# Symb0x76/ChineseChessZero

Measured on AMD Instinct MI355X. Metric: self-play MCTS simulations/sec, higher is better.
Workload: dtype u8 rules / f32 Q (reference CPU path) / f64 PUCT (net: fp16)

## Files before the change

chinesechesszero_amd/csrc/cczero.hip:

```cpp
#include "../../include/cczero.h"

#include <hip/hip_runtime.h>

#include <cmath>
#include <cstdarg>
#include <cstdio>
#include <cstdlib>
#include <cstddef>
#include <cstring>
#include <new>
#include <vector>

#include "cczero_kernels.h"
#include "cczero_history.h"
#include "cczero_mate.h"
#include "cczero_netops.h"
#include "cczero_conv.h"
#include "cczero_conv_small.h"
#include "cczero_conv_narrow.h"
#include "cczero_conv_g16.h"
#include "cczero_conv_g16e.h"
#include "cczero_heads.h"
#include "cczero_snapshot.h"

// ... 2302 lines not shown
    return 0;
}

int ccz_pack_conv_weights_g16_f16(void *stream, const void *w_dev, void *wp_dev, int32_t cin)
{
    if (!w_dev || !wp_dev || w_dev == wp_dev || (cin != 64 && cin != 128 && cin != 256)) return fail(-1, "ccz_pack_conv_weights_g16_f16: bad arguments (cin must be 64, 128 or 256, not in place)");
    if ((((uintptr_t)w_dev) | ((uintptr_t)wp_dev)) & 15) return fail(-1, "ccz_pack_conv_weights_g16_f16: pointers must be 16-byte aligned");
    const int n = 256 * 9 * (cin >> 3);
    hipLaunchKernelGGL(k_pack_conv_weights_g16, dim3((unsigned)((n + 255) / 256)), dim3(256), 0, (hipStream_t)stream, (const cv_half8 *)w_dev, (cv_half8 *)wp_dev, (int)cin);
    HIP_TRY(hipGetLastError());
    return 0;
}

int ccz_pack_live_planes_g16_f16(void *stream, const void *leaf_dev, void *x64_dev, int32_t n_boards, const int32_t *rows_dev, const int32_t *n_rows_dev)
{
    if (!leaf_dev || !x64_dev || n_boards < 0 || (!rows_dev) != (!n_rows_dev)) return fail(-1, "ccz_pack_live_planes_g16_f16: bad arguments");
    if ((uintptr_t)x64_dev & 15) return fail(-1, "ccz_pack_live_planes_g16_f16: output must be 16-byte aligned");
    if (n_boards == 0) return 0;
    hipLaunchKernelGGL(k_pack_live_planes, dim3((unsigned)n_boards), dim3(kPackThreads), 0, (hipStream_t)stream, (const _Float16 *)leaf_dev, (half8_t *)x64_dev, (int)n_boards,
                       (const int *)rows_dev, (const int *)n_rows_dev, rows_dev ? 3 : 1);
    HIP_TRY(hipGetLastError());
    return 0;
}

static int pack_planes128(const char *who, void *stream, const void *leaf_dev, void *x128_dev, int32_t n_boards, const int32_t *rows_dev, const int32_t *n_rows_dev, int flags)
{
    if (!leaf_dev || !x128_dev || n_boards < 0 || (!rows_dev) != (!n_rows_dev)) return fail(-1, "%s: bad arguments", who);
    if ((uintptr_t)x128_dev & 15) return fail(-1, "%s: output must be 16-byte aligned", who);
    if (n_boards == 0) return 0;
    hipLaunchKernelGGL(k_pack_planes128, dim3((unsigned)n_boards), dim3(kPackThreads), 0, (hipStream_t)stream, (const _Float16 *)leaf_dev, (half8_t *)x128_dev, (int)n_boards,
                       (const int *)rows_dev, (const int *)n_rows_dev, flags);
    HIP_TRY(hipGetLastError());
    return 0;
}

int ccz_pack_planes128_f16(void *stream, const void *leaf_dev, void *x128_dev, int32_t n_boards)
{
    return pack_planes128("ccz_pack_planes128_f16", stream, leaf_dev, x128_dev, n_boards, nullptr, nullptr, 0);
}

int ccz_pack_planes128_g16_f16(void *stream, const void *leaf_dev, void *x128_dev, int32_t n_boards, const int32_t *rows_dev, const int32_t *n_rows_dev)
{
    return pack_planes128("ccz_pack_planes128_g16_f16", stream, leaf_dev, x128_dev, n_boards, rows_dev, n_rows_dev, 1);
}

int ccz_pack_planes128_rows_f16(void *stream, const void *leaf_dev, void *x128_dev, int32_t n_boards, const int32_t *rows_dev, const int32_t *n_rows_dev)
{
    if (!rows_dev || !n_rows_dev) return fail(-1, "ccz_pack_planes128_rows_f16: bad arguments");
    return pack_planes128("ccz_pack_planes128_rows_f16", stream, leaf_dev, x128_dev, n_boards, rows_dev, n_rows_dev, 0);
}

int ccz_conv3x3_stem128_f16(void *stream, const void *x128_dev, const void *w_dev, const void *bias_f32_dev, void *y_dev, int64_t n_pixels, int32_t relu)
{
    if (relu & ~(3 | CCZ_CONV_G16)) return fail(-1, "ccz_conv3x3_stem128_f16: flags are ReLU (1), tile order (2) and CCZ_CONV_G16");
    return conv3x3_launch("ccz_conv3x3_stem128_f16", stream, x128_dev, w_dev, bias_f32_dev, nullptr, y_dev, n_pixels, relu, 128);
}

int ccz_conv3x3_stem128_f16_live(void *stream, const void *x128_dev, const void *w_dev, const void *bias_f32_dev, void *y_dev, int64_t n_pixels, int32_t relu,
                                 const int32_t *live_rows_dev, int32_t part, int32_t n_parts)
{
    if (relu & ~(3 | CCZ_CONV_G16)) return fail(-1, "ccz_conv3x3_stem128_f16_live: flags are ReLU (1), tile order (2) and CCZ_CONV_G16");
    if (!live_rows_dev || g16_bad_part(part, n_parts)) return fail(-1, "ccz_conv3x3_stem128_f16_live: null live-row count or bad part / n_parts");
    return conv3x3_launch("ccz_conv3x3_stem128_f16_live", stream, x128_dev, w_dev, bias_f32_dev, nullptr, y_dev, n_pixels, relu, 128, live_rows_dev, part | (n_parts << 16));
}

int ccz_pack_live_planes_f16(void *stream, const void *leaf_dev, void *x64_dev, int32_t n_boards)
{
    if (!leaf_dev || !x64_dev || n_boards < 0) return fail(-1, "ccz_pack_live_planes_f16: bad arguments");
    if ((uintptr_t)x64_dev & 15) return fail(-1, "ccz_pack_live_planes_f16: output must be 16-byte aligned");
    if (n_boards == 0) return 0;
    hipLaunchKernelGGL(k_pack_live_planes, dim3((unsigned)n_boards), dim3(kPackThreads), 0, (hipStream_t)stream, (const _Float16 *)leaf_dev, (half8_t *)x64_dev, (int)n_boards,
                       (const int *)nullptr, (const int *)nullptr, 0);
    HIP_TRY(hipGetLastError());
    return 0;
}

#ifdef CCZ_STAMPS
int ccz_debug_conv_stamps(unsigned long long *out_host)
{
    HIP_TRY(hipDeviceSynchronize());
    HIP_TRY(hipMemcpyFromSymbol(out_host, HIP_SYMBOL(g_cv_stamps), sizeof(unsigned long long) * 2048 * 2 * 16));
    return 0;
}
int ccz_debug_stamps(ccz_engine *e, void *stream, unsigned long long *out_host)
{
    NEED(e);
    hipStream_t s = (hipStream_t)stream;
    HIP_TRY(hipMemcpyAsync(out_host, e->d.stamps, (size_t)e->d.B * 16 * 8, hipMemcpyDeviceToHost, s));
    HIP_TRY(hipStreamSynchronize(s));
    return 0;
}
#endif

int ccz_heads_conv1x1_f16(void *stream, const void *x_dev, const void *w32_dev, const void *bias32_f32_dev, void *pol_dev, void *val_dev,
                          int32_t n_boards, int32_t flags, const int32_t *live_boards_dev)
{
    if (!x_dev || !w32_dev || !bias32_f32_dev || !pol_dev || !val_dev || n_boards < 0) return fail(-1, "ccz_heads_conv1x1_f16: bad arguments");
    if ((((uintptr_t)x_dev) | ((uintptr_t)w32_dev) | ((uintptr_t)bias32_f32_dev)) & 15) return fail(-1, "ccz_heads_conv1x1_f16: x, weights and bias must be 16-byte aligned");
    if (flags & ~CCZ_CONV_G16) return fail(-1, "ccz_heads_conv1x1_f16: unknown flags 0x%x", flags);
    const bool g16 = (flags & CCZ_CONV_G16) != 0;
    if (g16 && (n_boards & 15)) return fail(-1, "ccz_heads_conv1x1_f16: the group-of-16 layout holds whole groups of 16 boards (n_boards = %d)", n_boards);
    if (n_boards == 0) return 0;
    const long cells = ((long)n_boards * 90 + 15) / 16;
    const unsigned blocks = (unsigned)((cells + 3) / 4 < 768 ? (cells + 3) / 4 : 768);
    if (g16)
        hipLaunchKernelGGL(k_head_conv1x1<true>, dim3(blocks), dim3(256), 0, (hipStream_t)stream, (const _Float16 *)x_dev, (const _Float16 *)w32_dev,
                           (const float *)bias32_f32_dev, (_Float16 *)pol_dev, (_Float16 *)val_dev, (int)n_boards, (const int *)live_boards_dev);
    else
        hipLaunchKernelGGL(k_head_conv1x1<false>, dim3(blocks), dim3(256), 0, (hipStream_t)stream, (const _Float16 *)x_dev, (const _Float16 *)w32_dev,
                           (const float *)bias32_f32_dev, (_Float16 *)pol_dev, (_Float16 *)val_dev, (int)n_boards, (const int *)live_boards_dev);
    HIP_TRY(hipGetLastError());
    return 0;
}

static int conv3x3_cn_launch(const char *who, void *stream, const void *x_dev, const void *w_dev, const void *bias_f32_dev, const void *residual_dev, void *y_dev,
                             int64_t n_pixels, int32_t relu, int32_t cin, int32_t cout, const int32_t *live_rows_dev, int32_t row0)
{
    if ((cin != 64 && cin != 128) || (cout != 64 && cout != 128))
        return fail(-1, "%s: unsupported shape %d -> %d channels (cin and cout must be 64 or 128; 256-wide towers: ccz_conv3x3_c256_f16)", who, cin, cout);
    if (!x_dev || !w_dev || !bias_f32_dev || !y_dev || n_pixels < 0 || n_pixels > (int64_t)INT32_MAX / 256)
        return fail(-1, "%s: bad arguments (null pointer, or n_pixels outside 0 .. 2^31 / 256)", who);
    if ((((uintptr_t)x_dev) | ((uintptr_t)w_dev) | ((uintptr_t)bias_f32_dev) | ((uintptr_t)residual_dev) | ((uintptr_t)y_dev)) & 15)
        return fail(-1, "%s: pointers must be 16-byte aligned", who);
    if (x_dev == y_dev) return fail(-1, "%s: the output may alias the residual but not the input", who);
    if (relu & ~(CCZ_CONV_RELU | CCZ_CONV_DESCENDING | CCZ_CONV_FORCE_SMALL | CCZ_CONV_FORCE_TILE))
        return fail(-1, "%s: flags are ReLU, tile order and the two force bits (board-major rows only)", who);
    const bool whole = n_pixels % 90 == 0;
    if (live_rows_dev && !whole) return fail(-1, "%s: the live form takes whole boards (n_pixels = boards * 90)", who);
    if ((relu & CCZ_CONV_FORCE_SMALL) && (relu & CCZ_CONV_FORCE_TILE)) return fail(-1, "%s: both force bits set", who);
    if ((relu & CCZ_CONV_FORCE_SMALL) && (live_rows_dev || !whole)) return fail(-1, "%s: the small form takes whole boards and no live count", who);
    if (n_pixels == 0) return 0;
    const bool res = residual_dev != nullptr;
    const bool small = whole && !live_rows_dev && !(relu & CCZ_CONV_FORCE_TILE) && ((relu & CCZ_CONV_FORCE_SMALL) || n_pixels <= kSmallMaxPixels);
#define CCZ_CN_SMALL(RES_, CIN_, COUT_)                                                                                                         \
    hipLaunchKernelGGL((k_conv3x3_small<RES_, CIN_, COUT_>), dim3((unsigned)((n_pixels + kSmPix - 1) / kSmPix), COUT_ / 16), dim3(256), 0, (hipStream_t)stream, \
                       (const _Float16 *)x_dev, (const _Float16 *)w_dev, (const float *)bias_f32_dev, (const _Float16 *)residual_dev, (_Float16 *)y_dev, \
                       (int)n_pixels, (int)(relu & 1))
#define CCZ_CN_TILE(RES_, CIN_, COUT_)                                                                                                          \
    hipLaunchKernelGGL((k_conv3x3_narrow<RES_, CIN_, COUT_>), dim3((unsigned)((n_pixels + kNwBM - 1) / kNwBM)), dim3(512), 0, (hipStream_t)stream, \
                       (const _Float16 *)x_dev, (const _Float16 *)w_dev, (const float *)bias_f32_dev, (const _Float16 *)residual_dev, (_Float16 *)y_dev, \
                       (int)n_pixels, (int)(relu & 3), (const int *)live_rows_dev, (int)row0)
#define CCZ_CN_FORM(RES_, CIN_, COUT_) do { if (small) CCZ_CN_SMALL(RES_, CIN_, COUT_); else CCZ_CN_TILE(RES_, CIN_, COUT_); } while (0)
#define CCZ_CN_RES(CIN_, COUT_) do { if (res) CCZ_CN_FORM(true, CIN_, COUT_); else CCZ_CN_FORM(false, CIN_, COUT_); } while (0)
    if (cin == 64 && cout == 64) CCZ_CN_RES(64, 64);
    else if (cin == 64) CCZ_CN_RES(64, 128);
    else if (cout == 64) CCZ_CN_RES(128, 64);
    else CCZ_CN_RES(128, 128);
#undef CCZ_CN_RES
#undef CCZ_CN_FORM
#undef CCZ_CN_TILE
#undef CCZ_CN_SMALL
    HIP_TRY(hipGetLastError());
    return 0;
}

int ccz_conv3x3_cn_f16(void *stream, const void *x_dev, const void *w_dev, const void *bias_f32_dev, const void *residual_dev, void *y_dev,
                       int64_t n_pixels, int32_t relu, int32_t cin, int32_t cout)
{
    return conv3x3_cn_launch("ccz_conv3x3_cn_f16", stream, x_dev, w_dev, bias_f32_dev, residual_dev, y_dev, n_pixels, relu, cin, cout, nullptr, 0);
}

int ccz_conv3x3_cn_f16_live(void *stream, const void *x_dev, const void *w_dev, const void *bias_f32_dev, const void *residual_dev, void *y_dev,
                            int64_t n_pixels, int32_t relu, int32_t cin, int32_t cout, const int32_t *live_rows_dev, int32_t part, int32_t n_parts)
{
    if (!live_rows_dev || g16_bad_part(part, n_parts)) return fail(-1, "ccz_conv3x3_cn_f16_live: null live-row count or bad part / n_parts");
    return conv3x3_cn_launch("ccz_conv3x3_cn_f16_live", stream, x_dev, w_dev, bias_f32_dev, residual_dev, y_dev, n_pixels, relu, cin, cout, live_rows_dev,
// ... 78 lines not shown
```

chinesechesszero_amd/csrc/cczero_conv_g16.h:

```cpp
#pragma once
#include "cczero_conv.h"

namespace ccz {

constexpr int kG5Rows = 288;
constexpr int kG5SlabRows = 576;
constexpr int kG5SlabBytes = kG5SlabRows * 64;
constexpr int kG5WBytes = 256 * 64;
constexpr int kG5Ring = 5, kG5Ahead = 3;
constexpr int kG5AOff = kG5Ring * kG5WBytes;
constexpr int kG5Dump = kG5AOff + 2 * kG5SlabBytes;
constexpr int kG5Lds = kG5Dump + 8 * 1024;
constexpr int kG5ERow = 528;
static_assert(kG5Rows * kG5ERow <= kG5Dump, "epilogue image must fit the operand buffers");
constexpr int kG5QRows = 576;
constexpr int kG5QSlabRows = 864;
constexpr int kG5QSlabBytes = kG5QSlabRows * 64;
constexpr int kG5QWBytes = 128 * 64;
constexpr int kG5QAOff = kG5Ring * kG5QWBytes;
constexpr int kG5QDump = kG5QAOff + 2 * kG5QSlabBytes;
constexpr int kG5QLds = kG5QDump + 8 * 1024;
constexpr int kG5QERow = 272;
static_assert(kG5QLds == 159744 && kG5QLds <= kG5Lds, "quad tile: ring + two slabs + dump must fit the workgroup's LDS");
static_assert(kG5QRows * kG5QERow == 156672 && kG5QRows * kG5QERow <= kG5QLds,
              "quad tile: the epilogue image covers the operand buffers AND most of the dump area (free once every DMA has landed)");

constexpr int kG16CChunk = 1440 * 64;
__device__ __forceinline__ unsigned g16c_off(long p)
{
    const long g = p / 1440;
    return (unsigned)(g * (1440 * 512) + (p - g * 1440) * 64);
}

struct G5Ctx {
    unsigned char *lds;
    const _Float16 *X, *W;
    unsigned xbytes, wbytes;
    unsigned xbytes_part;
    unsigned xoff[5];
    unsigned xstep, whalf;
    unsigned woff;
    int zo[2], zd[2];
    int wave_dst;
    int lane16;
    int wave_dst_part, wave_step_part;
    int a_off;
    int vb[2];
    int cin, cmask;
};

__host__ __device__ constexpr bool g5_slab_tap(int t) { return t >= 1 && t <= 5; }
constexpr int kG5Split = 7;
__host__ __device__ constexpr int g5_dma(int t) { return 2 + (g5_slab_tap(t) ? 1 : 0); }
__host__ __device__ constexpr int g5_vmcnt(int t) { return g5_dma(t) + g5_dma(t - 1); }
static_assert(g5_vmcnt(0) == 4 && g5_vmcnt(1) == 5 && g5_vmcnt(2) == 6 && g5_vmcnt(3) == 6 && g5_vmcnt(4) == 6 && g5_vmcnt(5) == 6 &&
              g5_vmcnt(6) == 5 && g5_vmcnt(7) == 4 && g5_vmcnt(8) == 4, "g5_vmcnt table");
static_assert(g5_dma(0) == 2 && g5_dma(1) == 3 && g5_dma(2) == 3 && g5_dma(3) == 3 && g5_dma(4) == 3 && g5_dma(5) == 3 && g5_dma(6) == 2 &&
              g5_dma(7) == 2 && g5_dma(8) == 2, "23 DMA loads per chunk and thread: 5 slab pieces + 9 x 2 weight pieces");
__host__ __device__ constexpr int g5q_nslab(int t) { return t == 0 ? 2 : t <= 5 ? 1 : 0; }
__host__ __device__ constexpr int g5q_dma(int t) { return 1 + g5q_nslab(t); }
__host__ __device__ constexpr int g5q_vmcnt(int t) { return g5q_dma(t) + g5q_dma((t + 8) % 9); }
static_assert(g5q_vmcnt(0) == 4 && g5q_vmcnt(1) == 5 && g5q_vmcnt(2) == 4 && g5q_vmcnt(3) == 4 && g5q_vmcnt(4) == 4 && g5q_vmcnt(5) == 4 &&
              g5q_vmcnt(6) == 3 && g5q_vmcnt(7) == 2 && g5q_vmcnt(8) == 2, "g5q_vmcnt table");
static_assert(g5q_dma(0) == 3 && g5q_dma(1) == 2 && g5q_dma(2) == 2 && g5q_dma(3) == 2 && g5q_dma(4) == 2 && g5q_dma(5) == 2 && g5q_dma(6) == 1 &&
              g5q_dma(7) == 1 && g5q_dma(8) == 1, "16 DMA loads per chunk and thread: 7 slab pieces + 9 weight pieces");

template <int T, int N> __host__ __device__ constexpr bool g5_on_board()
{
    return !((T % 3 == 0 && N == 0) || (T % 3 == 2 && N == 8));
}

template <bool LDS_DONE = false> __device__ __forceinline__ void g5_barrier()
{
    if constexpr (LDS_DONE) asm volatile("s_waitcnt lgkmcnt(0)" ::: "memory");
    __builtin_amdgcn_sched_barrier(0);
    __builtin_amdgcn_s_barrier();
    __builtin_amdgcn_sched_barrier(0);
}

__device__ __forceinline__ void g5_zero_ranks(const G5Ctx &c, int buf)
{
    int l16 = c.lane16, zero = 0;
    asm volatile("" : "+v"(l16), "+v"(zero));
    typedef int g5_int4 __attribute__((ext_vector_type(4)));
    const g5_int4 z = {zero, zero, zero, zero};
#pragma unroll
    for (int j = 0; j < 2; ++j) *(g5_int4 *)(c.lds + (l16 + (c.zo[j] + buf * c.zd[j]))) = z;
    asm volatile("s_waitcnt lgkmcnt(0)" ::: "memory");
}

#define G5_CELL(TAP, N)                                                                                                   \
    {                                                                                                                     \
        if constexpr (TAP % 3 == 2)                                                                                       \
            b[N] = *(const cv_half8 *)(lds + c.vb[BUFn] + G5_REFILL(N) * 1024);                                           \
        if constexpr (g5_on_board<TAP, N>()) {                                                                            \
            constexpr int NB = N + TAP % 3 - 1;                                                                           \
            _Pragma("unroll") for (int i = 0; i < 4; ++i)                                                                 \
                acc[i][N] = __builtin_amdgcn_mfma_f32_16x16x32_f16(acur[i], b[NB], acc[i][N], 0, 0, 0);                   \
        }                                                                                                                 \
        __builtin_amdgcn_sched_barrier(0);                                                                                \
    }
#define G5_CELLS(TAP, LO, HI)                                                                                             \
    if constexpr (LO <= 0 && 0 < HI) G5_CELL(TAP, 0) if constexpr (LO <= 1 && 1 < HI) G5_CELL(TAP, 1) if constexpr (LO <= 2 && 2 < HI) G5_CELL(TAP, 2) \
    if constexpr (LO <= 3 && 3 < HI) G5_CELL(TAP, 3) if constexpr (LO <= 4 && 4 < HI) G5_CELL(TAP, 4) if constexpr (LO <= 5 && 5 < HI) G5_CELL(TAP, 5) \
    if constexpr (LO <= 6 && 6 < HI) G5_CELL(TAP, 6) if constexpr (LO <= 7 && 7 < HI) G5_CELL(TAP, 7) if constexpr (LO <= 8 && 8 < HI) G5_CELL(TAP, 8)

template <int J, bool Q = false, bool CM = false>
__device__ __forceinline__ void g5_step(const G5Ctx &c, cv_f32x4 (&acc)[4][9], int chunk, int &ring_rd, int &ring_wr,
                                         cv_half8 (&a0)[4], cv_half8 (&a1)[4], cv_half8 (&b)[9])
{
    constexpr int T = J % 9, BUF = J / 9;
    constexpr int Tn = (T + 1) % 9, BUFn = (T == 8) ? 1 - BUF : BUF;
    constexpr int kWB = Q ? kG5QWBytes : kG5WBytes, kAOff = Q ? kG5QAOff : kG5AOff, kSlab = Q ? kG5QSlabBytes : kG5SlabBytes;
    cv_half8 (&acur)[4] = (J & 1) ? a1 : a0;
    cv_half8 (&anxt)[4] = (J & 1) ? a0 : a1;
    unsigned char *const lds = c.lds;

#define G5_REFILL(N) (9 + N + 9 * (Tn / 3 - 1))
    constexpr int T2 = (T + kG5Ahead) % 9;
    const int chunk2 = chunk + (T + kG5Ahead >= 9 ? 1 : 0);
    G5_CELLS(T, 0, 1)
    if constexpr (Q && g5q_nslab(T) > 0) {
        constexpr int pass = T == 0 ? 0 : T + 1;
        const unsigned so = (unsigned)((chunk + 1) * (CM ? kG16CChunk : 64));
        const unsigned live = chunk < c.cmask ? (pass < 6 ? c.xbytes : c.xbytes_part) : 0u;
        cv_blds16(c.X, live, c.xoff[0], so + pass * c.xstep,
                  lds + (pass < 6 ? kAOff + (1 - BUF) * kSlab + pass * 8192 + c.wave_dst : c.wave_dst_part + (1 - BUF) * c.wave_step_part));
        if constexpr (g5q_nslab(T) > 1) cv_blds16(c.X, live, c.xoff[0], so + (pass + 1) * c.xstep, lds + kAOff + (1 - BUF) * kSlab + ((pass + 1) * 8192 + c.wave_dst));
        __builtin_amdgcn_sched_barrier(0);
    }
    if constexpr (!Q && g5_dma(T) > 2) {
        constexpr int pass = T - 1;
        const unsigned live = pass < 4 ? c.xbytes : c.xbytes_part;
        cv_blds16(c.X, chunk < c.cmask ? live : 0u, c.xoff[pass], (unsigned)((chunk + 1) * (CM ? kG16CChunk : 64)),
                  lds + (pass < 4 ? kG5AOff + (1 - BUF) * kG5SlabBytes + pass * 8192 + c.wave_dst : c.wave_dst_part + (1 - BUF) * c.wave_step_part));
        __builtin_amdgcn_sched_barrier(0);
    }
    G5_CELLS(T, 1, 2)
    if constexpr (Q) {
        cv_blds16(c.W, chunk2 <= c.cmask ? c.wbytes : 0u, c.woff, (unsigned)((T2 + 9 * chunk2) * (2 * 8192)) + c.whalf, lds + ring_wr * kWB + c.wave_dst);
        __builtin_amdgcn_sched_barrier(0);
        G5_CELLS(T, 2, 3)
    } else {
        const unsigned wlive = chunk2 <= c.cmask ? c.wbytes : 0u;
        const unsigned so = (unsigned)((T2 + 9 * chunk2) * (2 * 8192));
        unsigned char *const d = lds + ring_wr * kG5WBytes + c.wave_dst;
        cv_blds16(c.W, wlive, c.woff, so, d);
        __builtin_amdgcn_sched_barrier(0);
        G5_CELLS(T, 2, 3)
        cv_blds16(c.W, wlive, c.woff, so + 8192u, d + 8192);
        __builtin_amdgcn_sched_barrier(0);
    }
    G5_CELLS(T, 3, kG5Split)

    ring_rd = ring_rd + 1 == kG5Ring ? 0 : ring_rd + 1;
    cv_wait_vm<Q ? g5q_vmcnt(T) : g5_vmcnt(T)>();
    if constexpr (!Q && T == 7) g5_zero_ranks(c, 1 - BUF);
    g5_barrier();

    {
        const unsigned char *wa = lds + (ring_rd * kWB + c.a_off);
#pragma unroll
        for (int i = 0; i < 4; ++i) anxt[i] = *(const cv_half8 *)(wa + i * 1024);
        __builtin_amdgcn_sched_barrier(0);
    }
    G5_CELLS(T, kG5Split, 9)
    ring_wr = ring_wr + 1 == kG5Ring ? 0 : ring_wr + 1;
#undef G5_REFILL
}

struct G5Heads {
    const _Float16 *w32;
    const float *b32;
    _Float16 *pol, *val;
    int nb;
};

__device__ __forceinline__ void g5_heads_phase(const unsigned char *lds, int w, int lane, const G5Heads &ha, const long (&board0)[2],
                                               const int (&pos0)[2], bool skip1)
{
    const int r = lane & 15, q4 = lane >> 4;
    cv_half8 a[2][8];
#pragma unroll
    for (int m = 0; m < 2; ++m)
#pragma unroll
        for (int s = 0; s < 8; ++s) a[m][s] = *(const cv_half8 *)(ha.w32 + (m * 16 + r) * 256 + s * 32 + q4 * 8);
    const float4 b0 = *(const float4 *)(ha.b32 + 4 * q4), b1 = *(const float4 *)(ha.b32 + 16 + 4 * q4);
    for (int cell = w; cell < 18; cell += 8) {
        const unsigned char *row = lds + (cell * 16 + r) * kG5ERow + q4 * 16;
        cv_f32x4 acc0, acc1;
        acc0[0] = b0.x; acc0[1] = b0.y; acc0[2] = b0.z; acc0[3] = b0.w;
        acc1[0] = b1.x; acc1[1] = b1.y; acc1[2] = b1.z; acc1[3] = b1.w;
#pragma unroll
        for (int s = 0; s < 8; ++s) {
            const cv_half8 b = *(const cv_half8 *)(row + s * 64);
            acc0 = __builtin_amdgcn_mfma_f32_16x16x32_f16(a[0][s], b, acc0, 0, 0, 0);
            acc1 = __builtin_amdgcn_mfma_f32_16x16x32_f16(a[1][s], b, acc1, 0, 0, 0);
        }
        const int wnr = cell >= 9 ? 1 : 0, n = cell - 9 * wnr;
        const long board = board0[wnr] + r;
        if (board < ha.nb && !(skip1 && wnr)) {
            const int pos = pos0[wnr] + n;
            _Float16 *po = ha.pol + board * 1536 + pos * 17;
            _Float16 *vo = ha.val + board * 640 + pos * 7;
#pragma unroll
            for (int e = 0; e < 4; ++e) po[4 * q4 + e] = (_Float16)fmaxf(acc0[e], 0.0f);
            if (q4 == 0) {
                po[16] = (_Float16)fmaxf(acc1[0], 0.0f);
                vo[0] = (_Float16)fmaxf(acc1[1], 0.0f);
                vo[1] = (_Float16)fmaxf(acc1[2], 0.0f);
                vo[2] = (_Float16)fmaxf(acc1[3], 0.0f);
            } else if (q4 == 1) {
#pragma unroll
                for (int e = 0; e < 4; ++e) vo[3 + e] = (_Float16)fmaxf(acc1[e], 0.0f);
            }
        }
    }
}

__device__ __forceinline__ int g5_live_groups(const int *live_rows, int row0, int cap, int &first)
{
    const int part = row0 & 0xffff, n_parts = row0 >> 16;
    const int G = (*live_rows + 15) >> 4;
    const int per = (G + n_parts - 1) / n_parts;
    first = part * per;
    int live = G - first;
    live = live < 0 ? 0 : (live > per ? per : live);
    return live > cap ? cap : live;
}

template <bool RES, bool HEADS>
__device__ __forceinline__ void g5_live_part(int first, int cin, const _Float16 *__restrict__ &X, const _Float16 *&R, _Float16 *&Y, long &first_board)
{
    const long off = (long)first * 1440 * kCvC;
    X += (long)first * 1440 * cin;
    if (!HEADS) Y += off;
    if (RES) R += off;
    first_board = (long)first * 16;
}

__device__ __forceinline__ int g5_xcd_tile(int blk, int tiles, int flags)
{
    const int b = blk, x = b & 7, per = tiles >> 3, rem = tiles & 7;
    const int tile = x * per + (x < rem ? x : rem) + (b >> 3);
    return __builtin_amdgcn_readfirstlane((flags & 2) ? tiles - 1 - tile : tile);
}

__device__ __forceinline__ void g5_ctx_common(G5Ctx &c, unsigned char *lds, const _Float16 *X, const _Float16 *W, int w, unsigned xbytes, int cin, int chunks)
{
    c.lds = lds;
// ... 144 lines not shown
    cv_wait_vm<4>();
    g5_zero_ranks(c, 0);
    g5_barrier<true>();

    int ring_rd = 0, ring_wr = kG5Ahead;
    cv_half8 a0[4], a1[4], b[9];
#pragma unroll
    for (int i = 0; i < 4; ++i) a0[i] = *(const cv_half8 *)(lds + c.a_off + i * 1024);
#pragma unroll
    for (int n = 0; n < 9; ++n) b[n] = *(const cv_half8 *)(lds + c.vb[0] + (9 + n - 9) * 1024);
#define G5_S(j) g5_step<j, false, CM && !ONE>(c, acc, chunk + (j) / 9, ring_rd, ring_wr, a0, a1, b)
    if constexpr (ONE) {
        const int chunk = 0;
        G5_S(0); G5_S(1); G5_S(2); G5_S(3); G5_S(4); G5_S(5); G5_S(6); G5_S(7); G5_S(8);
    } else {
        for (int chunk = 0; chunk <= c.cmask; chunk += 2) {
            G5_S(0); G5_S(1); G5_S(2); G5_S(3); G5_S(4); G5_S(5); G5_S(6); G5_S(7); G5_S(8);
            G5_S(9); G5_S(10); G5_S(11); G5_S(12); G5_S(13); G5_S(14); G5_S(15); G5_S(16); G5_S(17);
        }
    }
#undef G5_S
    cv_wait_vm<0>();

    g5_barrier();
    const int lane_e = (int)__builtin_amdgcn_mbcnt_hi(~0u, __builtin_amdgcn_mbcnt_lo(~0u, 0u));
    const int re = lane_e & 15, q4e = lane_e >> 4;
    const int prow = lane_e >> 5, piece = lane_e & 31;
    const long pbase = p0 + w * 36 + prow;
    cv_half8 rv[18];
    g5_image_store<kG5ERow>(lds, acc, wm, wn, re, q4e);
    if constexpr (CM) {
        const int erow = g16c_lane_row(lane_e), ep = lane_e & 3;
        const size_t yo = (size_t)g16c_off(p0 + erow) + (size_t)(w * kG16CChunk + ep * 16);
        if (RES) {
#pragma unroll
            for (int it = 0; it < 18; ++it) rv[it] = *(const cv_half8 *)((const unsigned char *)R + yo + it * 1024);
        }
        g5_barrier<true>();
        g5c_rows_out<kG5ERow, RES, HEADS>(lds, erow * kG5ERow + w * 64 + ep * 16, yo, Y, relu, rv);
    } else {
        if (RES) {
#pragma unroll
            for (int it = 0; it < 18; ++it) rv[it] = *(const cv_half8 *)(R + (pbase + it * 2) * kCvC + piece * 8);
        }
        g5_barrier<true>();
        g5_rows_out<kG5ERow, 2, RES, HEADS>(lds, w * 36 + prow, piece, pbase, piece * 8, Y, relu, rv);
    }
    if constexpr (HEADS) {
        g5_barrier<true>();
        const long grp = p0 / 1440;
        const int rank0 = (int)((p0 - grp * 1440) / 144);
        const long board0[2] = {first_board + grp * 16, first_board + grp * 16};
        const int pos0[2] = {rank0 * 9, rank0 * 9 + 9};
        g5_heads_phase(lds, w, lane_e, ha, board0, pos0, false);
    }
}

template <bool RES, bool CM = false>
__device__ __forceinline__ void g5q_tile(unsigned char *lds, int blk, int grid, const _Float16 *__restrict__ X, const _Float16 *__restrict__ W,
                                         const float *__restrict__ bias, const _Float16 *R, _Float16 *Y, int M, int relu, int cin,
                                         const int *live_rows, int row0)
{
    const int tid = threadIdx.x, lane = tid & 63;
    const int w = __builtin_amdgcn_readfirstlane(tid >> 6);
    const int r = lane & 15, q4 = lane >> 4;
    const int wm = w & 1, wn = w >> 1;
    int tiles = grid;
    if (live_rows) {
        int first;
        const int live = g5_live_groups(live_rows, row0, M / 1440, first);
        M = live * 1440;
        tiles = live * 4;
        if (blk >= tiles) return;
        long first_board;
        g5_live_part<RES, false>(first, cin, X, R, Y, first_board);
    }
    const int tile = g5_xcd_tile(blk, tiles, relu);
    const int h = tile & 1;
    const long p0 = (long)(tile >> 2) * 1440 + 144 + (long)((tile >> 1) & 1) * kG5QRows;
    relu &= 1;

    G5Ctx c;
    g5_ctx_common(c, lds, X, W, w, (unsigned)M * (unsigned)cin * 2u, cin, cin >> 5);
    c.wave_dst_part = w < 6 ? kG5QAOff + 6 * 8192 + w * 1024 : kG5QDump + w * 1024;
    c.wave_step_part = w < 6 ? kG5QSlabBytes : 0;
    c.xbytes_part = w < 6 ? c.xbytes : 0u;
    c.xstep = CM ? 128u * 64u : 128u * (unsigned)cin * 2u;
    c.whalf = (unsigned)h * 8192u;
    {
        const int sr = tid >> 2, pos = tid & 3;
        const int schunk = pos ^ ((0 - (sr >> 2)) & 3);
        if constexpr (CM) c.xoff[0] = g16c_off(p0 - 144 + sr) + (unsigned)(schunk * 16);
        else c.xoff[0] = (unsigned)((p0 - 144 + sr) * cin + schunk * 8) * 2u;
        c.woff = (unsigned)(tid * 16);
    }
#pragma unroll
    for (int it = 0; it < 7; ++it)
        cv_blds16(X, it < 6 ? c.xbytes : c.xbytes_part, c.xoff[0], it * c.xstep, lds + (it < 6 ? kG5QAOff + it * 8192 + c.wave_dst : c.wave_dst_part));
#pragma unroll
    for (int u = 0; u < kG5Ahead; ++u) cv_blds16(W, c.wbytes, c.woff, (unsigned)(u * 2 * 8192) + c.whalf, lds + u * kG5QWBytes + c.wave_dst);
    g5_ctx_frags(c, r, q4, wm, wn * 9, kG5QAOff, kG5QSlabBytes);

    cv_f32x4 acc[4][9];
#pragma unroll
    for (int i = 0; i < 4; ++i) g5_acc_row_from_bias(acc[i], bias + h * 128 + wm * 64 + i * 16 + 4 * q4);

    cv_wait_vm<2>();
    g5_barrier();

    int ring_rd = 0, ring_wr = kG5Ahead;
    cv_half8 a0[4], a1[4], b[9];
#pragma unroll
    for (int i = 0; i < 4; ++i) a0[i] = *(const cv_half8 *)(lds + c.a_off + i * 1024);
#pragma unroll
    for (int n = 0; n < 9; ++n) b[n] = *(const cv_half8 *)(lds + c.vb[0] + n * 1024);
    for (int chunk = 0; chunk <= c.cmask; chunk += 2) {
#define G5Q_S(j) g5_step<j, true, CM>(c, acc, chunk + (j) / 9, ring_rd, ring_wr, a0, a1, b)
        G5Q_S(0); G5Q_S(1); G5Q_S(2); G5Q_S(3); G5Q_S(4); G5Q_S(5); G5Q_S(6); G5Q_S(7); G5Q_S(8);
        G5Q_S(9); G5Q_S(10); G5Q_S(11); G5Q_S(12); G5Q_S(13); G5Q_S(14); G5Q_S(15); G5Q_S(16); G5Q_S(17);
#undef G5Q_S
    }
    cv_wait_vm<0>();

    g5_barrier();
    const int lane_e = (int)__builtin_amdgcn_mbcnt_hi(~0u, __builtin_amdgcn_mbcnt_lo(~0u, 0u));
    const int re = lane_e & 15, q4e = lane_e >> 4;
    const int prow = lane_e >> 4, piece = lane_e & 15;
    const long pbase = p0 + w * 72 + prow;
    const int gcol = h * 128 + piece * 8;
    cv_half8 rv[18];
    g5_image_store<kG5QERow>(lds, acc, wm, wn, re, q4e);
    if constexpr (CM) {
        const int erow = g16c_lane_row(lane_e), ep = lane_e & 3, ch = w & 3, irow = (w >> 2) * 288 + erow;
        const size_t yo = (size_t)g16c_off(p0 + irow) + (size_t)((h * 4 + ch) * kG16CChunk + ep * 16);
        if (RES) {
#pragma unroll
            for (int it = 0; it < 18; ++it) rv[it] = *(const cv_half8 *)((const unsigned char *)R + yo + it * 1024);
        }
        g5_barrier<true>();
        g5c_rows_out<kG5QERow, RES, false>(lds, irow * kG5QERow + ch * 64 + ep * 16, yo, Y, relu, rv);
    } else {
        if (RES) {
#pragma unroll
            for (int it = 0; it < 18; ++it) rv[it] = *(const cv_half8 *)(R + (pbase + it * 4) * kCvC + gcol);
        }
        g5_barrier<true>();
        g5_rows_out<kG5QERow, 4, RES, false>(lds, w * 72 + prow, piece, pbase, gcol, Y, relu, rv);
    }
}

template <bool RES>
__global__ __launch_bounds__(512) void k_conv3x3_g16(const _Float16 *__restrict__ X, const _Float16 *__restrict__ W,
                                                         const float *__restrict__ bias, const _Float16 *R,
                                                         _Float16 *Y, int M, int relu, int cin, const int *live_rows, int row0)
{
    __shared__ __attribute__((aligned(16))) unsigned char lds[kG5Lds];
    g5_tile<RES, false>(lds, blockIdx.x, gridDim.x, X, W, bias, R, Y, M, relu, cin, live_rows, row0, G5Heads{});
}

template <bool RES>
__global__ __launch_bounds__(512) void k_conv3x3_g16_quad(const _Float16 *__restrict__ X, const _Float16 *__restrict__ W,
                                                            const float *__restrict__ bias, const _Float16 *R,
                                                            _Float16 *Y, int M, int relu, int cin, const int *live_rows, int row0)
{
    __shared__ __attribute__((aligned(16))) unsigned char lds[kG5Lds];
    g5q_tile<RES>(lds, blockIdx.x, gridDim.x, X, W, bias, R, Y, M, relu, cin, live_rows, row0);
}

__global__ __launch_bounds__(512) void k_conv3x3_g16_stem(const _Float16 *__restrict__ X, const _Float16 *__restrict__ W,
                                                            const float *__restrict__ bias, _Float16 *Y, int M, int relu, int cin,
                                                            const int *live_rows, int row0)
{
    __shared__ __attribute__((aligned(16))) unsigned char lds[kG5Lds];
    g5_tile<false, false, true>(lds, blockIdx.x, gridDim.x, X, W, bias, nullptr, Y, M, relu, cin, live_rows, row0, G5Heads{});
}

__global__ __launch_bounds__(512) void k_conv3x3_g16_heads(const _Float16 *__restrict__ X, const _Float16 *__restrict__ W,
                                                             const float *__restrict__ bias, const _Float16 *R, _Float16 *Y, int M,
                                                             int relu, int cin, const int *live_rows, int row0, G5Heads ha)
{
    __shared__ __attribute__((aligned(16))) unsigned char lds[kG5Lds];
    if (live_rows) ha.nb = *live_rows;
    g5_tile<true, true>(lds, blockIdx.x, gridDim.x, X, W, bias, R, Y, M, relu, cin, live_rows, row0, ha);
}

__global__ __launch_bounds__(512) void k_conv3x3_g16c_stem(const _Float16 *__restrict__ X, const _Float16 *__restrict__ W,
                                                             const float *__restrict__ bias, _Float16 *Y, int M, int relu, int cin,
                                                             const int *live_rows, int row0)
{
    __shared__ __attribute__((aligned(16))) unsigned char lds[kG5Lds];
    g5_tile<false, false, true, true>(lds, blockIdx.x, gridDim.x, X, W, bias, nullptr, Y, M, relu, cin, live_rows, row0, G5Heads{});
}

__global__ __launch_bounds__(512) void k_conv3x3_g16c_heads(const _Float16 *__restrict__ X, const _Float16 *__restrict__ W,
                                                              const float *__restrict__ bias, const _Float16 *R, _Float16 *Y, int M,
                                                              int relu, int cin, const int *live_rows, int row0, G5Heads ha)
{
    __shared__ __attribute__((aligned(16))) unsigned char lds[kG5Lds];
    if (live_rows) ha.nb = *live_rows;
    g5_tile<true, true, false, true>(lds, blockIdx.x, gridDim.x, X, W, bias, R, Y, M, relu, cin, live_rows, row0, ha);
}

__global__ __launch_bounds__(256) void k_pack_conv_weights_g16(const cv_half8 *__restrict__ w, cv_half8 *__restrict__ wp, int cin)
{
// ... 10 lines not shown
```

Baseline: 201,300.

## Halve quad-tile conv barriers by pairing half-steps with a six-slot weight ring

The quad-tile 3x3 conv main loop now waits and issues a workgroup barrier only on every second tap step. It grows the weight ring from five to six slots and prefetches four steps ahead, so that ring slots are compile-time functions of the step. Slab DMA issue is rescheduled across the 18 half-steps so each wait count still covers the data needed. This cuts barrier and vmcnt stall overhead in exchange for 2KB more LDS and deeper prefetch, with the dump area shifted for some waves. Stamp instrumentation and profiling scripts are added behind a compile flag.

```diff
diff --git a/chinesechesszero_amd/csrc/cczero.hip b/chinesechesszero_amd/csrc/cczero.hip
--- a/chinesechesszero_amd/csrc/cczero.hip
+++ b/chinesechesszero_amd/csrc/cczero.hip
@@ -2408,6 +2408,17 @@
     HIP_TRY(hipMemcpyFromSymbol(out_host, HIP_SYMBOL(g_cv_stamps), sizeof(unsigned long long) * 2048 * 2 * 16));
     return 0;
 }
+int ccz_debug_g5q_stamps(unsigned long long *out_host, int clear)
+{
+    HIP_TRY(hipDeviceSynchronize());
+    HIP_TRY(hipMemcpyFromSymbol(out_host, HIP_SYMBOL(g_g5q_stamps), sizeof(unsigned long long) * 4096 * 8 * 8));
+    if (clear) {
+        void *p = nullptr;
+        HIP_TRY(hipGetSymbolAddress(&p, HIP_SYMBOL(g_g5q_stamps)));
+        HIP_TRY(hipMemset(p, 0, sizeof(unsigned long long) * 4096 * 8 * 8));
+    }
+    return 0;
+}
 int ccz_debug_stamps(ccz_engine *e, void *stream, unsigned long long *out_host)
 {
     NEED(e);
diff --git a/chinesechesszero_amd/csrc/cczero_conv_g16.h b/chinesechesszero_amd/csrc/cczero_conv_g16.h
--- a/chinesechesszero_amd/csrc/cczero_conv_g16.h
+++ b/chinesechesszero_amd/csrc/cczero_conv_g16.h
@@ -17,13 +17,19 @@
 constexpr int kG5QSlabRows = 864;
 constexpr int kG5QSlabBytes = kG5QSlabRows * 64;
 constexpr int kG5QWBytes = 128 * 64;
-constexpr int kG5QAOff = kG5Ring * kG5QWBytes;
+#ifndef CCZ_G5Q_PAIR
+#define CCZ_G5Q_PAIR 1
+#endif
+constexpr bool kG5QPair = CCZ_G5Q_PAIR != 0;
+constexpr int kG5QRing = kG5QPair ? 6 : kG5Ring, kG5QAhead = kG5QPair ? 4 : kG5Ahead;
+constexpr int kG5QAOff = kG5QRing * kG5QWBytes;
 constexpr int kG5QDump = kG5QAOff + 2 * kG5QSlabBytes;
-constexpr int kG5QLds = kG5QDump + 8 * 1024;
+constexpr int kG5QDumpWave0 = kG5QPair ? 6 : 0;
+constexpr int kG5QLds = kG5QDump + (8 - kG5QDumpWave0) * 1024;
 constexpr int kG5QERow = 272;
-static_assert(kG5QLds == 159744 && kG5QLds <= kG5Lds, "quad tile: ring + two slabs + dump must fit the workgroup's LDS");
+static_assert(kG5QLds == (kG5QPair ? 161792 : 159744) && kG5QLds <= kG5Lds, "quad tile: ring + two slabs + dump must fit the workgroup's LDS");
 static_assert(kG5QRows * kG5QERow == 156672 && kG5QRows * kG5QERow <= kG5QLds,
-              "quad tile: the epilogue image covers the operand buffers AND most of the dump area (free once every DMA has landed)");
+              "quad tile: the epilogue image covers the operand buffers (ring of five: and most of the dump area), free once every DMA has landed");
 
 constexpr int kG16CChunk = 1440 * 64;
 __device__ __forceinline__ unsigned g16c_off(long p)
@@ -47,6 +53,9 @@
     int a_off;
     int vb[2];
     int cin, cmask;
+#ifdef CCZ_STAMPS
+    mutable unsigned long long st_vm, st_bar, st_n;
+#endif
 };
 
 __host__ __device__ constexpr bool g5_slab_tap(int t) { return t >= 1 && t <= 5; }
@@ -65,6 +74,17 @@
 static_assert(g5q_dma(0) == 3 && g5q_dma(1) == 2 && g5q_dma(2) == 2 && g5q_dma(3) == 2 && g5q_dma(4) == 2 && g5q_dma(5) == 2 && g5q_dma(6) == 1 &&
               g5q_dma(7) == 1 && g5q_dma(8) == 1, "16 DMA loads per chunk and thread: 7 slab pieces + 9 weight pieces");
 
+__host__ __device__ constexpr int g5q2_nslab(int j) { return j < 9 ? g5q_nslab(j) : j - 9 <= 1 ? 2 : j - 9 <= 4 ? 1 : 0; }
+__host__ __device__ constexpr int g5q2_pass(int j) { return j % 9 == 0 ? 0 : g5q2_pass(j - 1) + g5q2_nslab(j - 1); }
+__host__ __device__ constexpr int g5q2_dma(int j) { return 1 + g5q2_nslab(j); }
+__host__ __device__ constexpr int g5q2_vmcnt(int j) { return g5q2_dma(j) + g5q2_dma((j + 17) % 18); }
+__host__ __device__ constexpr bool g5q2_barrier(int j) { return (j & 1) != 0; }
+static_assert(g5q2_vmcnt(1) == 5 && g5q2_vmcnt(3) == 4 && g5q2_vmcnt(5) == 4 && g5q2_vmcnt(7) == 2 && g5q2_vmcnt(9) == 4 && g5q2_vmcnt(11) == 5 &&
+              g5q2_vmcnt(13) == 4 && g5q2_vmcnt(15) == 2 && g5q2_vmcnt(17) == 2, "g5q2_vmcnt table (the odd half-steps wait)");
+static_assert(g5q2_pass(8) == 7 && g5q2_pass(17) == 7 && g5q2_pass(5) == 6 && g5q2_pass(13) == 6 && g5q2_nslab(6) == 0 && g5q2_nslab(14) == 0,
+              "seven slab pieces per chunk; the last one is issued in J = 5 resp. 13, two half-steps in front of the barriers of J = 7 resp. 15");
+static_assert(18 % kG5QRing == 0 || !kG5QPair, "the slot of a half-step is a compile-time function of J");
+
 template <int T, int N> __host__ __device__ constexpr bool g5_on_board()
 {
     return !((T % 3 == 0 && N == 0) || (T % 3 == 2 && N == 8));
@@ -77,6 +97,15 @@
     __builtin_amdgcn_s_barrier();
     __builtin_amdgcn_sched_barrier(0);
 }
+
+#ifdef CCZ_STAMPS
+__device__ unsigned long long g_g5q_stamps[4096 * 8 * 8];
+#define G5Q_STAMP(s_) const unsigned long long s_ = cv_stamp();
+#define G5Q_STAMP_ADD(c_, s0_, s1_, s2_) (c_).st_vm += s1_ - s0_; (c_).st_bar += s2_ - s1_; (c_).st_n += 1;
+#else
+#define G5Q_STAMP(s_)
+#define G5Q_STAMP_ADD(c_, s0_, s1_, s2_)
+#endif
 
 __device__ __forceinline__ void g5_zero_ranks(const G5Ctx &c, int buf)
 {
@@ -117,16 +146,19 @@
     unsigned char *const lds = c.lds;
 
 #define G5_REFILL(N) (9 + N + 9 * (Tn / 3 - 1))
-    constexpr int T2 = (T + kG5Ahead) % 9;
-    const int chunk2 = chunk + (T + kG5Ahead >= 9 ? 1 : 0);
+    constexpr bool P = Q && kG5QPair;
+    constexpr int kAhead = Q ? kG5QAhead : kG5Ahead;
+    constexpr int T2 = (T + kAhead) % 9;
+    const int chunk2 = chunk + (T + kAhead >= 9 ? 1 : 0);
+    constexpr int nslab = !Q ? 0 : P ? g5q2_nslab(J) : g5q_nslab(T);
     G5_CELLS(T, 0, 1)
-    if constexpr (Q && g5q_nslab(T) > 0) {
-        constexpr int pass = T == 0 ? 0 : T + 1;
+    if constexpr (nslab > 0) {
+        constexpr int pass = P ? g5q2_pass(J) : T == 0 ? 0 : T + 1;
         const unsigned so = (unsigned)((chunk + 1) * (CM ? kG16CChunk : 64));
         const unsigned live = chunk < c.cmask ? (pass < 6 ? c.xbytes : c.xbytes_part) : 0u;
         cv_blds16(c.X, live, c.xoff[0], so + pass * c.xstep,
                   lds + (pass < 6 ? kAOff + (1 - BUF) * kSlab + pass * 8192 + c.wave_dst : c.wave_dst_part + (1 - BUF) * c.wave_step_part));
-        if constexpr (g5q_nslab(T) > 1) cv_blds16(c.X, live, c.xoff[0], so + (pass + 1) * c.xstep, lds + kAOff + (1 - BUF) * kSlab + ((pass + 1) * 8192 + c.wave_dst));
+        if constexpr (nslab > 1) cv_blds16(c.X, live, c.xoff[0], so + (pass + 1) * c.xstep, lds + kAOff + (1 - BUF) * kSlab + ((pass + 1) * 8192 + c.wave_dst));
         __builtin_amdgcn_sched_barrier(0);
     }
     if constexpr (!Q && g5_dma(T) > 2) {
@@ -138,7 +170,8 @@
     }
     G5_CELLS(T, 1, 2)
     if constexpr (Q) {
-        cv_blds16(c.W, chunk2 <= c.cmask ? c.wbytes : 0u, c.woff, (unsigned)((T2 + 9 * chunk2) * (2 * 8192)) + c.whalf, lds + ring_wr * kWB + c.wave_dst);
+        if constexpr (P) cv_blds16(c.W, chunk2 <= c.cmask ? c.wbytes : 0u, c.woff, (unsigned)((T2 + 9 * chunk2) * (2 * 8192)) + c.whalf, lds + ((J + kAhead) % kG5QRing) * kWB + c.wave_dst);
+        else cv_blds16(c.W, chunk2 <= c.cmask ? c.wbytes : 0u, c.woff, (unsigned)((T2 + 9 * chunk2) * (2 * 8192)) + c.whalf, lds + ring_wr * kWB + c.wave_dst);
         __builtin_amdgcn_sched_barrier(0);
         G5_CELLS(T, 2, 3)
     } else {
@@ -153,19 +186,38 @@
     }
     G5_CELLS(T, 3, kG5Split)
 
-    ring_rd = ring_rd + 1 == kG5Ring ? 0 : ring_rd + 1;
-    cv_wait_vm<Q ? g5q_vmcnt(T) : g5_vmcnt(T)>();
-    if constexpr (!Q && T == 7) g5_zero_ranks(c, 1 - BUF);
-    g5_barrier();
-
-    {
-        const unsigned char *wa = lds + (ring_rd * kWB + c.a_off);
+    if constexpr (P) {
+        if constexpr (g5q2_barrier(J)) {
+            G5Q_STAMP(s0)
+            cv_wait_vm<g5q2_vmcnt(J)>();
+            G5Q_STAMP(s1)
+            g5_barrier();
+            G5Q_STAMP(s2)
+            G5Q_STAMP_ADD(c, s0, s1, s2)
+        } else __builtin_amdgcn_sched_barrier(0);
+        const unsigned char *wa = lds + (((J + 1) % kG5QRing) * kWB + c.a_off);
 #pragma unroll
         for (int i = 0; i < 4; ++i) anxt[i] = *(const cv_half8 *)(wa + i * 1024);
         __builtin_amdgcn_sched_barrier(0);
-    }
-    G5_CELLS(T, kG5Split, 9)
-    ring_wr = ring_wr + 1 == kG5Ring ? 0 : ring_wr + 1;
+        G5_CELLS(T, kG5Split, 9)
+    } else {
+        ring_rd = ring_rd + 1 == kG5Ring ? 0 : ring_rd + 1;
+        if constexpr (Q) { G5Q_STAMP(s0) cv_wait_vm<g5q_vmcnt(T)>(); G5Q_STAMP(s1) g5_barrier(); G5Q_STAMP(s2) G5Q_STAMP_ADD(c, s0, s1, s2) }
+        else {
+            cv_wait_vm<g5_vmcnt(T)>();
+            if constexpr (T == 7) g5_zero_ranks(c, 1 - BUF);
+            g5_barrier();
+        }
+
+        {
+            const unsigned char *wa = lds + (ring_rd * kWB + c.a_off);
+#pragma unroll
+            for (int i = 0; i < 4; ++i) anxt[i] = *(const cv_half8 *)(wa + i * 1024);
+            __builtin_amdgcn_sched_barrier(0);
+        }
+        G5_CELLS(T, kG5Split, 9)
+        ring_wr = ring_wr + 1 == kG5Ring ? 0 : ring_wr + 1;
+    }
 #undef G5_REFILL
 }
 
@@ -476,7 +528,7 @@
 
     G5Ctx c;
     g5_ctx_common(c, lds, X, W, w, (unsigned)M * (unsigned)cin * 2u, cin, cin >> 5);
-    c.wave_dst_part = w < 6 ? kG5QAOff + 6 * 8192 + w * 1024 : kG5QDump + w * 1024;
+    c.wave_dst_part = w < 6 ? kG5QAOff + 6 * 8192 + w * 1024 : kG5QDump + (w - kG5QDumpWave0) * 1024;
     c.wave_step_part = w < 6 ? kG5QSlabBytes : 0;
     c.xbytes_part = w < 6 ? c.xbytes : 0u;
     c.xstep = CM ? 128u * 64u : 128u * (unsigned)cin * 2u;
@@ -492,7 +544,7 @@
     for (int it = 0; it < 7; ++it)
         cv_blds16(X, it < 6 ? c.xbytes : c.xbytes_part, c.xoff[0], it * c.xstep, lds + (it < 6 ? kG5QAOff + it * 8192 + c.wave_dst : c.wave_dst_part));
 #pragma unroll
-    for (int u = 0; u < kG5Ahead; ++u) cv_blds16(W, c.wbytes, c.woff, (unsigned)(u * 2 * 8192) + c.whalf, lds + u * kG5QWBytes + c.wave_dst);
+    for (int u = 0; u < kG5QAhead; ++u) cv_blds16(W, c.wbytes, c.woff, (unsigned)(u * 2 * 8192) + c.whalf, lds + u * kG5QWBytes + c.wave_dst);
     g5_ctx_frags(c, r, q4, wm, wn * 9, kG5QAOff, kG5QSlabBytes);
 
     cv_f32x4 acc[4][9];
@@ -502,18 +554,33 @@
     cv_wait_vm<2>();
     g5_barrier();
 
-    int ring_rd = 0, ring_wr = kG5Ahead;
+    int ring_rd = 0, ring_wr = kG5QAhead;
     cv_half8 a0[4], a1[4], b[9];
 #pragma unroll
     for (int i = 0; i < 4; ++i) a0[i] = *(const cv_half8 *)(lds + c.a_off + i * 1024);
 #pragma unroll
     for (int n = 0; n < 9; ++n) b[n] = *(const cv_half8 *)(lds + c.vb[0] + n * 1024);
+#ifdef CCZ_STAMPS
+    c.st_vm = c.st_bar = c.st_n = 0;
+    const unsigned long long st_loop0 = cv_stamp(), st_real0 = __builtin_amdgcn_s_memrealtime();
+    __builtin_amdgcn_s_waitcnt(0xC07F);
+#endif
     for (int chunk = 0; chunk <= c.cmask; chunk += 2) {
 #define G5Q_S(j) g5_step<j, true, CM>(c, acc, chunk + (j) / 9, ring_rd, ring_wr, a0, a1, b)
         G5Q_S(0); G5Q_S(1); G5Q_S(2); G5Q_S(3); G5Q_S(4); G5Q_S(5); G5Q_S(6); G5Q_S(7); G5Q_S(8);
         G5Q_S(9); G5Q_S(10); G5Q_S(11); G5Q_S(12); G5Q_S(13); G5Q_S(14); G5Q_S(15); G5Q_S(16); G5Q_S(17);
 #undef G5Q_S
     }
+#ifdef CCZ_STAMPS
+    {
+        const unsigned long long st_loop1 = cv_stamp(), st_real1 = __builtin_amdgcn_s_memrealtime();
+        __builtin_amdgcn_s_waitcnt(0xC07F);
+        if (blk < 4096 && lane == 0) {
+            unsigned long long *o = g_g5q_stamps + ((size_t)blk * 8 + w) * 8;
+            o[0] = c.st_vm; o[1] = c.st_bar; o[2] = st_loop1 - st_loop0; o[3] = st_real1 - st_real0; o[4] = c.st_n;
+        }
+    }
+#endif
     cv_wait_vm<0>();
 
     g5_barrier();
diff --git a/profiles/conv_quad_stamps.py b/profiles/conv_quad_stamps.py
--- /dev/null
+++ b/profiles/conv_quad_stamps.py
@@ -0,0 +1,82 @@
+import argparse
+import ctypes as C
+import json
+import os
+import sys
+import time
+
+import numpy as np
+
+ROOT = os.path.dirname(os.path.dirname(os.path.abspath(__file__)))
+FLAGS = 1 | 64 | 128 | 512 | 65536
+LIBS = (("pair", "libcczero_stamps.so"), ("ring5", "libcczero_stamps_ring5.so"))
+
+
+def main():
+    ap = argparse.ArgumentParser()
+    ap.add_argument("--boards", type=int, nargs="+", default=[4096, 3696])
+    ap.add_argument("--seconds", type=float, default=2.5)
+    ap.add_argument("--libdir", default=os.path.join(ROOT, "build", "diag"), help="where the two diagnostic libraries are")
+    ap.add_argument("--out")
+    a = ap.parse_args()
+    import torch
+    sys.path.insert(0, ROOT)
+    from chinesechesszero_amd.net import g16_to_g16c, pack_conv_weights_g16
+    dev = torch.device("cuda:0")
+    s = C.c_void_p(torch.cuda.current_stream().cuda_stream)
+    result = {"flags": FLAGS, "seconds": a.seconds, "half_steps": 72, "stamp_cost_note": "a stamp is about 40 cycles; each wait and each barrier segment holds one",
+              "layers": []}
+    libs = []
+    for name, f in LIBS:
+        p = os.path.join(a.libdir, f)
+        if os.path.exists(p):
+            L = C.CDLL(p)
+            L.ccz_conv3x3_c256_g16c_f16.restype = C.c_int
+            L.ccz_conv3x3_c256_g16c_f16.argtypes = [C.c_void_p] * 6 + [C.c_int64, C.c_int32]
+            L.ccz_debug_g5q_stamps.restype = C.c_int
+            L.ccz_debug_g5q_stamps.argtypes = [C.c_void_p, C.c_int]
+            libs.append((name, L))
+    assert libs, "no diagnostic library in " + a.libdir
+    for B in a.boards:
+        G = B // 16
+        g = torch.Generator(device="cpu").manual_seed(1)
+        x = g16_to_g16c(torch.relu(torch.randn(G, 1440, 256, generator=g) * 0.5).to(dev).half())
+        res = g16_to_g16c(torch.relu(torch.randn(G, 1440, 256, generator=g) * 0.5).to(dev).half())
+        w = (torch.randn(256, 3, 3, 256, generator=g) * 0.03).to(dev).half()
+        bias = (torch.randn(256, generator=g) * 0.1).to(dev)
+        wp = pack_conv_weights_g16(w)
+        y = torch.zeros_like(x)
+        layer = {"boards": B, "quad_workgroups": G * 4}
+        for name, L in libs:
+            st = np.zeros(4096 * 8 * 8, np.uint64)
+            assert L.ccz_debug_g5q_stamps(st.ctypes.data_as(C.c_void_p), 1) == 0
+            t0, n = time.time(), 0
+            while time.time() - t0 < a.seconds:
+                for _ in range(200):
+                    assert L.ccz_conv3x3_c256_g16c_f16(s, x.data_ptr(), wp.data_ptr(), bias.data_ptr(), res.data_ptr(), y.data_ptr(), B * 90, FLAGS) == 0
+                torch.cuda.synchronize()
+                n += 200
+            assert L.ccz_debug_g5q_stamps(st.ctypes.data_as(C.c_void_p), 0) == 0
+            v = st.reshape(4096, 8, 8)[:min(4096, G * 4)].astype(np.float64)
+            vm, bar, loop, real, meet = (v[:, :, i] for i in range(5))
+            assert (meet > 0).all()
+            med = lambda t: float(np.median(t))
+            layer[name] = {
+                "launches": n, "meetings_per_tile": med(meet),
+                "vmcnt_wait_cycles_per_meeting": med(vm / meet), "barrier_cycles_per_meeting": med(bar / meet),
+                "vmcnt_wait_cycles_per_half_step": med(vm / 72), "barrier_cycles_per_half_step": med(bar / 72),
+                "half_step_cycles": med(loop / 72), "loop_cycles": med(loop),
+                "wait_plus_barrier_share_of_loop": med((vm + bar) / loop),
+                "wait_plus_barrier_share_less_stamps": med((vm + bar - 80 * meet) / (loop - 120 * meet)),
+                "slowest_wave_over_fastest_barrier_cycles": med(bar.max(axis=1) / np.maximum(bar.min(axis=1), 1)),
+                "clock_ghz": med(loop / np.maximum(real, 1)) * 0.1,
+            }
+        result["layers"].append(layer)
+    txt = json.dumps(result, indent=1)
+    print(txt)
+    if a.out:
+        open(a.out, "w").write(txt + "\n")
+
+
+if __name__ == "__main__":
+    main()
diff --git a/profiles/quad_barrier_layer_ab.py b/profiles/quad_barrier_layer_ab.py
--- /dev/null
+++ b/profiles/quad_barrier_layer_ab.py
@@ -0,0 +1,85 @@
+import argparse
+import ctypes as C
+import json
+import os
+import statistics
+import sys
+
+ROOT = os.path.dirname(os.path.dirname(os.path.abspath(__file__)))
+FLAGS = 1 | 64 | 128 | 512 | 65536
+
+
+def main():
+    ap = argparse.ArgumentParser()
+    ap.add_argument("other")
+    ap.add_argument("--boards", type=int, nargs="+", default=[4096, 3696])
+    ap.add_argument("--rounds", type=int, default=7)
+    ap.add_argument("--iters", type=int, default=100)
+    ap.add_argument("--out")
+    a = ap.parse_args()
+    import torch
+    sys.path.insert(0, ROOT)
+    from chinesechesszero_amd.net import g16_to_g16c, g16c_to_g16, pack_conv_weights_g16
+
+    def load(path):
+        L = C.CDLL(os.path.abspath(path))
+        for f in ("ccz_conv3x3_c256_f16", "ccz_conv3x3_c256_g16c_f16"):
+            getattr(L, f).restype = C.c_int
+            getattr(L, f).argtypes = [C.c_void_p] * 6 + [C.c_int64, C.c_int32]
+        return L
+
+    ring5, pair = load(a.other), load(os.path.join(ROOT, "chinesechesszero_amd", "libcczero.so"))
+    dev = torch.device("cuda:0")
+    s = C.c_void_p(torch.cuda.current_stream().cuda_stream)
+    result = {"flags": FLAGS, "rounds": a.rounds, "iters": a.iters, "layers": []}
+    for B in a.boards:
+        G = B // 16
+        g = torch.Generator(device="cpu").manual_seed(1)
+        x = torch.relu(torch.randn(G, 1440, 256, generator=g) * 0.5).to(dev).half()
+        res = torch.relu(torch.randn(G, 1440, 256, generator=g) * 0.5).to(dev).half()
+        w = (torch.randn(256, 3, 3, 256, generator=g) * 0.03).to(dev).half()
+        bias = (torch.randn(256, generator=g) * 0.1).to(dev)
+        wp = pack_conv_weights_g16(w)
+        xc, rc = g16_to_g16c(x), g16_to_g16c(res)
+        arms = [("ring5_rows", ring5.ccz_conv3x3_c256_f16, x, res), ("pair_rows", pair.ccz_conv3x3_c256_f16, x, res),
+                ("ring5_g16c", ring5.ccz_conv3x3_c256_g16c_f16, xc, rc), ("pair_g16c", pair.ccz_conv3x3_c256_g16c_f16, xc, rc)]
+        ys = [torch.zeros_like(x) for _ in arms]
+
+        def run(i):
+            _, fn, xin, rin = arms[i]
+            assert fn(s, xin.data_ptr(), wp.data_ptr(), bias.data_ptr(), rin.data_ptr(), ys[i].data_ptr(), B * 90, FLAGS) == 0
+
+        for i in range(len(arms)):
+            run(i)
+        torch.cuda.synchronize()
+        same = [bool(torch.equal(g16c_to_g16(y) if n.endswith("g16c") else y, ys[0])) for (n, *_), y in zip(arms, ys)]
+        assert all(same), "outputs differ"
+        for _ in range(3):
+            for i in range(len(arms)):
+                for _ in range(a.iters):
+                    run(i)
+        torch.cuda.synchronize()
+        times = {n: [] for n, *_ in arms}
+        for rnd in range(a.rounds):
+            order = list(range(len(arms)))
+            order = order[rnd % len(arms):] + order[:rnd % len(arms)]
+            for i in order:
+                e0, e1 = torch.cuda.Event(enable_timing=True), torch.cuda.Event(enable_timing=True)
+                run(i)
+                e0.record()
+                for _ in range(a.iters):
+                    run(i)
+                e1.record()
+                torch.cuda.synchronize()
+                times[arms[i][0]].append(e0.elapsed_time(e1) / a.iters * 1e3)
+        us = {n: {"median": statistics.median(t), "min": min(t), "max": max(t), "all": [round(v, 2) for v in t]} for n, t in times.items()}
+        result["layers"].append({"boards": B, "outputs_identical": same, "nonzero_out": int((ys[0] != 0).sum().item()), "us": us,
+                                 "pair_over_ring5_median": {k: us["pair_" + k]["median"] / us["ring5_" + k]["median"] for k in ("rows", "g16c")}})
+    txt = json.dumps(result, indent=1)
+    print(txt)
+    if a.out:
+        open(a.out, "w").write(txt + "\n")
+
+
+if __name__ == "__main__":
+    main()
```

New measurement: 204,800, median of 6. 1.7% higher.
